# jltsiren/bwt-merge

Measured on AMD Instinct MI355X. Metric: merged Gbases/sec (input1+input2), bit-exact native BWT; value = inputs and result resident in HBM, host_to_host_value = SURVEY 8(d)'s T (page-locked host to page-locked host), higher is better.
Workload: dtype u64

## Files before the change

### bwt-merge_amd/csrc/api/context.hip.h

```cpp
#pragma once


namespace
{

thread_local std::string g_error;

int fail(int code, const char* fmt, ...)
{
  char buf[512];
  va_list ap; va_start(ap, fmt); vsnprintf(buf, sizeof(buf), fmt, ap); va_end(ap);
  g_error = buf;
  return code;
}

inline u64 div_up(u64 a, u64 b) { return (a + b - 1) / b; }

}


struct bwtm_context
{
  int device = -1;
  hipStream_t stream = nullptr;
// ... 3 lines not shown
  std::atomic<long long> live_handles{0};

  bool profiling = false;
  std::string profile_only;
  bool profile_open = false;
  struct Pending { const char* name; hipEvent_t start, stop; };
  std::vector<Pending> pending;
  std::map<std::string, std::pair<double, uint64_t>> totals;
  std::vector<const char*> order;

  std::multimap<u64, void*> free_blocks;
  u64 cached_bytes = 0, held_bytes = 0, peak_bytes = 0;
  struct VBlock { u64 bytes = 0; std::vector<hipMemGenericAllocationHandle_t> chunks; hipEvent_t released = nullptr; };
  bool vmm = false;
  std::vector<hipMemGenericAllocationHandle_t> free_chunks;
  std::map<void*, VBlock> vblocks;
  u64 device_total = 0;
  u64 va_fallbacks = 0;

  void* stream_stage[4] = {nullptr, nullptr, nullptr, nullptr};
  u64 stream_stage_cap[4] = {0, 0, 0, 0};
  u64* host_scratch = nullptr;
  u64 scan1_tiles = 0, pull_scan1_tiles = 0;
  u64 step_forms[3] = {0, 0, 0};
  u64 transcode_forms[16] = {};
};

namespace
{

struct Tuning
{
  long long search_algo = 0;
  long long frontier_unfused = 0;
  long long l1_cap = 0;
  long long emit_path = 0;
  long long round_emits = 1ll << 33;
  long long emit_budget = 0;
  long long frontier_epoch = 512;
  long long eager_cum_budget = 16ll << 30;
  long long upload_chunk = 256ll << 20;
  long long download_chunk = 128ll << 20;
  long long range_ratio = 8;
#ifdef BWTM_EXPERIMENTAL
  long long search_view = 0;
#endif
  long long frontier_stage_out = 1;
  long long frontier_rel = 1;
  long long frontier_parts = 0;
  long long part_capacity = 0;
  long long recs_uniform = 0;
  long long recs_window = 0;
  long long stream_samples_query = 0;
  long long stream_upload = 0;
  long long extract_batch = 1ll << 20;
  long long locate_batch = 1ll << 20;
  long long overlap_batch = 1ll << 20;
  long long approx_batch = 1ll << 16;
  long long correct_batch = 1ll << 20;
  long long ingest_verify = 0;
#ifdef BWTM_DIAGNOSTICS
  long long walk_emit = 0;
  long long walk_blocks = 0;
  long long walk_kernel = 0;
  long long walk_ablate = 0;
  long long walk_variant = 0;
// ... 25 lines not shown
  for(int k = 0; k < 4; k++) { if(c->stream_stage[k]) { (void)hipHostFree(c->stream_stage[k]); } c->stream_stage[k] = nullptr; c->stream_stage_cap[k] = 0; }
}
void apply_env_tuning();

int context_setup(bwtm_context* c, int device)
{
  int count = 0;
  hipError_t e = hipGetDeviceCount(&count);
  if(e != hipSuccess || count <= 0) { return fail(BWTM_ENODEV, "no HIP device available (%s)", hipGetErrorString(e)); }
  if(device < 0 || device >= count) { return fail(BWTM_EINVAL, "device %d out of range (%d devices)", device, count); }
  HIP_TRY(hipSetDevice(device));
  apply_env_tuning();
  c->device = device;
  HIP_TRY(hipStreamCreateWithFlags(&c->stream, hipStreamNonBlocking));
  HIP_TRY(hipStreamCreateWithFlags(&c->copy_stream, hipStreamNonBlocking));
  HIP_TRY(hipHostMalloc((void**)&c->host_scratch, 128 * sizeof(u64), hipHostMallocDefault));
  vmm_setup(c);
  {
    hipDeviceProp_t prop;
    HIP_TRY(hipGetDeviceProperties(&prop, device));
    int per_cu_scan = 0, per_cu_pull = 0;
    HIP_TRY(hipOccupancyMaxActiveBlocksPerMultiprocessor(&per_cu_scan, (const void*)k_frontier_scan1, BLOCK_THREADS, 0));
    HIP_TRY(hipOccupancyMaxActiveBlocksPerMultiprocessor(&per_cu_pull, (const void*)k_pull_scan1, BLOCK_THREADS, 0));
    c->scan1_tiles = std::min<u64>(FRONTIER_SCAN1_TILES, (u64)std::max(per_cu_scan, 0) * (u64)std::max(prop.multiProcessorCount, 0));
    c->pull_scan1_tiles = std::min<u64>(FRONTIER_SCAN1_TILES, (u64)std::max(per_cu_pull, 0) * (u64)std::max(prop.multiProcessorCount, 0));
  }
  HIP_TRY(hipFuncSetAttribute((const void*)k_part_scatter_sorted, hipFuncAttributeMaxDynamicSharedMemorySize, 96 * 1024));
  HIP_TRY(hipFuncSetAttribute((const void*)k_lf_walk_binned<true>, hipFuncAttributeMaxDynamicSharedMemorySize, 40 * 1024));
#ifdef BWTM_DIAGNOSTICS
  HIP_TRY(hipFuncSetAttribute((const void*)k_lf_walk_lds<true>, hipFuncAttributeMaxDynamicSharedMemorySize, 122 * 1024));
  HIP_TRY(hipFuncSetAttribute((const void*)k_lf_walk_lds<false>, hipFuncAttributeMaxDynamicSharedMemorySize, 82 * 1024));
#endif
  return BWTM_OK;
}

void context_teardown(bwtm_context* c)
{
  if(c->device < 0) { return; }
  (void)hipSetDevice(c->device);
  if(c->stream) { (void)hipStreamSynchronize(c->stream); }
  if(c->copy_stream) { (void)hipStreamSynchronize(c->copy_stream); }
  for(auto& p : c->pending) { (void)hipEventDestroy(p.start); (void)hipEventDestroy(p.stop); }
  c->pending.clear();
  pool_trim(c);
  stream_stage_free(c);
  if(c->host_scratch) { (void)hipHostFree(c->host_scratch); }
// ... 40 lines not shown
      ctx->mu.unlock();
    }
  }
  Scope(const Scope&) = delete; Scope& operator=(const Scope&) = delete;
};

#define ENTER(wanted) Scope scope_(wanted); if(scope_.rc != BWTM_OK) { return scope_.rc; }


void profile_begin(const char* name)
{
  CTX.profile_open = (CTX.profiling && (CTX.profile_only.empty() || CTX.profile_only.find(std::string(",") + name + ",") != std::string::npos));
  if(!CTX.profile_open) { return; }
  bwtm_context::Pending p; p.name = name;
  (void)hipEventCreate(&p.start); (void)hipEventCreate(&p.stop);
  (void)hipEventRecord(p.start, CTX.stream);
  CTX.pending.push_back(p);
}

void profile_end()
{
  if(!CTX.profile_open) { return; }
  (void)hipEventRecord(CTX.pending.back().stop, CTX.stream);
}

void profile_collect()
{
  if(CTX.pending.empty()) { return; }
  (void)hipStreamSynchronize(CTX.stream);
  for(auto& p : CTX.pending)
  {
    float ms = 0; (void)hipEventElapsedTime(&ms, p.start, p.stop);
    auto it = CTX.totals.find(p.name);
    if(it == CTX.totals.end()) { CTX.totals[p.name] = std::make_pair((double)ms, (uint64_t)1); CTX.order.push_back(p.name); }
    else { it->second.first += ms; it->second.second += 1; }
    (void)hipEventDestroy(p.start); (void)hipEventDestroy(p.stop);
  }
  CTX.pending.clear();
}

#define LAUNCH_CFG(name, kernel, gridx, gridy, block, lds, ...) do { \
  const unsigned long long gx_ = (unsigned long long)(gridx); \
  if(gx_ * (unsigned long long)(block) >= (1ull << 32)) { return fail(BWTM_EINVAL, "launch of %s: %llu workgroups of %u threads do not fit one grid", name, gx_, (unsigned)(block)); } \
  profile_begin(name); \
  hipLaunchKernelGGL(kernel, dim3((unsigned)gx_, (unsigned)(gridy)), dim3((unsigned)(block)), (unsigned)(lds), CTX.stream, __VA_ARGS__); \
  profile_end(); \
// ... 357 lines not shown
  {
    fail(BWTM_EINVAL, "bwtm_context_destroy: %lld handles of the context are still alive; context not destroyed", context->live_handles.load());
    return;
  }
  context_teardown(context);
  delete context;
}

extern "C" const char* bwtm_last_error(void) { return g_error.c_str(); }

namespace
{
int tune_set(const char* key, long long value)
{
  std::string k(key);
  if(k == "search_algo") { g_tune.search_algo = value; }
  else if(k == "frontier_unfused") { g_tune.frontier_unfused = value; }
  else if(k == "l1_cap") { g_tune.l1_cap = value; }
  else if(k == "emit_path") { g_tune.emit_path = value; }
  else if(k == "round_emits") { g_tune.round_emits = (value > 0 ? value : 1); }
  else if(k == "emit_budget") { g_tune.emit_budget = (value > 0 ? value : 0); }
  else if(k == "frontier_epoch") { g_tune.frontier_epoch = (value > 0 ? value : 512); }
  else if(k == "range_ratio") { g_tune.range_ratio = (value >= 0 ? value : 8); }
#ifdef BWTM_EXPERIMENTAL
  else if(k == "search_view") { g_tune.search_view = (value >= 0 && value <= 2 ? value : 0); }
#endif
  else if(k == "frontier_stage_out") { g_tune.frontier_stage_out = (value != 0); }
  else if(k == "frontier_rel") { g_tune.frontier_rel = (value >= 0 && value <= 2 ? value : 1); }
  else if(k == "frontier_parts") { g_tune.frontier_parts = (value > 0 ? value : 0); }
  else if(k == "stream_samples_query") { g_tune.stream_samples_query = (value != 0); }
  else if(k == "stream_upload") { g_tune.stream_upload = (value != 0); }
  else if(k == "ingest_verify") { g_tune.ingest_verify = (value != 0); }
  else if(k == "extract_batch") { g_tune.extract_batch = (value > 0 ? value : (1ll << 20)); }
  else if(k == "locate_batch") { g_tune.locate_batch = (value > 0 ? std::min<long long>(value, 1ll << 28) : (1ll << 20)); }
  else if(k == "overlap_batch") { g_tune.overlap_batch = (value > 0 ? std::min<long long>(value, 1ll << 28) : (1ll << 20)); }
  else if(k == "approx_batch") { g_tune.approx_batch = (value > 0 ? std::min<long long>(value, 1ll << 28) : (1ll << 16)); }
  else if(k == "correct_batch") { g_tune.correct_batch = (value > 0 ? std::min<long long>(value, 1ll << 28) : (1ll << 20)); }
  else if(k == "part_capacity") { g_tune.part_capacity = value; }
  else if(k == "recs_uniform") { g_tune.recs_uniform = (value > 0 ? 1 : (value < 0 ? -1 : 0)); }
  else if(k == "recs_window") { g_tune.recs_window = (value == 8192 || value == 16384 || value == 32768 ? value : 0); }
  else if(k == "eager_cum_budget") { g_tune.eager_cum_budget = (value > 0 ? value : (16ll << 30)); }
  else if(k == "upload_chunk") { g_tune.upload_chunk = (value > 0 ? value : (256ll << 20)); }
  else if(k == "download_chunk") { g_tune.download_chunk = (value > 0 ? value : (128ll << 20)); }
#ifdef BWTM_DIAGNOSTICS
  else if(k == "walk_emit") { g_tune.walk_emit = value; }
  else if(k == "walk_blocks") { g_tune.walk_blocks = value; }
// ... 165 lines not shown
```

### bwt-merge_amd/csrc/api/search.hip.h

```cpp
#pragma once

struct bwtm_ra
{
  bwtm_context* ctx = nullptr;
  bwtm_ra() : ctx(t_ctx) { if(ctx) { ctx->live_handles++; } }
  ~bwtm_ra() { if(ctx) { ctx->live_handles--; } }
  bwtm_ra(const bwtm_ra&) = delete; bwtm_ra& operator=(const bwtm_ra&) = delete;
  u64 na = 0, nb = 0, n_out = 0;
  u64 nrecs_out = 0, nchunks = 0;
  DevBuf owned_bits;
  void* bits_ptr = nullptr;
  template<class T> T* bits_as() const { return (T*)bits_ptr; }
  DevBuf chunk_base;
  bool finalized = false;
  u64 values = 0;
  bool ranged = false;
  u64 range_first = 0, range_last = 0;
  DevBuf range_rel;
  DevBuf super_boff;
  bool windowed = false;
  u64 win_word_first = 0, win_words = 0;
};

#define WHOLE_RA(ra, who) if((ra)->windowed) { return fail(BWTM_EINVAL, who ": a window of a rank array (bwtm_ra_create_range) only serves the merge over partitioned records and the output-range entry points"); }
// ... 184 lines not shown
  DevBuf segmin; TRY(segmin.alloc(nsteps * nsegs * sizeof(u32)));
  LAUNCH2D("bound_seg_min", k_bound_seg_min, nsegs, nsteps, BLOCK_THREADS, bound.as<const u32>(), ntiles, nsegs, segmin.as<u32>());
  LAUNCH2D("bound_suffix_min", k_bound_suffix_min, nsegs, nsteps, BLOCK_THREADS, bound.as<u32>(), ntiles, nsegs, segmin.as<const u32>(), emit_base.as<const u64>());
  LAUNCH("tile_build", k_tile_build_frontier, ntiles, BLOCK_THREADS, emit16.as<const unsigned short>(), emit_base.as<const u64>(), emit_cap, bound.as<const u32>(),
    ntiles, nsteps, ra->bits_as<u64>() + (tile_first << (TILE_SHIFT - 6)), ra->nchunks * CHUNK_WORDS - (tile_first << (TILE_SHIFT - 6)));
  return BWTM_OK;
}

struct RangeLevels
{
  DevBuf sp[2], r[2], cnt[2], flags, pieces, npieces;
  u64 N = 0, alive = 0, levels = 0;
  u32 piece_cap = 0;
  int cur = 0;
  void release() { for(int k = 0; k < 2; k++) { sp[k].release(); r[k].release(); cnt[k].release(); } flags.release(); pieces.release(); npieces.release(); }
};

int range_phase(const bwtm_index* a, const bwtm_index* b, u64 seq_first, u64 count, bwtm_ra* ra, u64 limit, RangeLevels& L)
{
  const u64 cap = std::min<u64>(5 * limit, count) + 1;
  for(int k = 0; k < 2; k++) { TRY(L.sp[k].alloc(cap * sizeof(u64))); TRY(L.r[k].alloc(cap * sizeof(u64))); TRY(L.cnt[k].alloc(cap * sizeof(u64))); }
  TRY(L.flags.alloc((5 * limit + 1) * sizeof(u64)));
  L.piece_cap = (u32)std::min<u64>(count / 16 + 1024, 1ull << 24);
  TRY(L.pieces.alloc((u64)L.piece_cap * sizeof(RangePiece)));
  TRY(L.npieces.alloc(sizeof(u32), true));
  LAUNCH("range_init", k_range_init, 1, BLOCK_THREADS, L.sp[0].as<u64>(), L.r[0].as<u64>(), L.cnt[0].as<u64>(), seq_first, count, a->m);
  L.N = 1; L.alive = count; L.cur = 0; L.levels = 0;
  while(L.N > 0 && L.N <= limit)
  {
    const int c = L.cur;
    const u64 N = L.N, grid = div_up(N, BLOCK_THREADS);
    LAUNCH("range_step", k_range_step<false>, grid, BLOCK_THREADS, a->view(), b->view(), L.sp[c].as<const u64>(), L.r[c].as<const u64>(), L.cnt[c].as<const u64>(), N,
      L.flags.as<u64>(), (const u64*)nullptr, (u64*)nullptr, (u64*)nullptr, (u64*)nullptr, ra->bits_as<u32>(), L.pieces.as<RangePiece>(), L.npieces.as<u32>(), L.piece_cap);
    LAUNCH("range_emit", k_range_emit, 2048, BLOCK_THREADS, L.pieces.as<const RangePiece>(), L.npieces.as<const u32>(), L.piece_cap, ra->bits_as<u32>());
    HIP_TRY(hipMemsetAsync(L.npieces.p, 0, sizeof(u32), CTX.stream));
    TRY(device_scan<0>(L.flags.as<u64>(), L.flags.as<u64>(), 5 * N + 1));
    LAUNCH("range_children", k_range_step<true>, grid, BLOCK_THREADS, a->view(), b->view(), L.sp[c].as<const u64>(), L.r[c].as<const u64>(), L.cnt[c].as<const u64>(), N,
      (u64*)nullptr, L.flags.as<const u64>(), L.sp[1 - c].as<u64>(), L.r[1 - c].as<u64>(), L.cnt[1 - c].as<u64>(), (u32*)nullptr, (RangePiece*)nullptr, (u32*)nullptr, 0u);
    TRY(fetch_u64(L.flags.as<u64>() + 5 * N, 0));
    HIP_TRY(hipStreamSynchronize(CTX.stream));
    L.N = CTX.host_scratch[0];
    L.cur = 1 - c; L.levels++;
  }
  return BWTM_OK;
}

int range_alive(RangeLevels& L, DevBuf& offsets)
{
  TRY(offsets.alloc((L.N + 1) * sizeof(u64)));
  HIP_TRY(hipMemcpyAsync(offsets.p, L.cnt[L.cur].p, L.N * sizeof(u64), hipMemcpyDeviceToDevice, CTX.stream));
  HIP_TRY(hipMemsetAsync(offsets.as<u64>() + L.N, 0, sizeof(u64), CTX.stream));
  TRY(device_scan<0>(offsets.as<u64>(), offsets.as<u64>(), L.N + 1));
  TRY(fetch_u64(offsets.as<u64>() + L.N, 0));
  HIP_TRY(hipStreamSynchronize(CTX.stream));
  L.alive = CTX.host_scratch[0];
  return BWTM_OK;
}

int range_expand(RangeLevels& L, const DevBuf& offsets, uint2* lo, unsigned short* hi)
{
  const int c = L.cur;
  LAUNCH("range_expand", k_range_expand, div_up(L.N, BLOCK_THREADS), BLOCK_THREADS, L.sp[c].as<const u64>(), L.r[c].as<const u64>(), L.cnt[c].as<const u64>(),
    offsets.as<const u64>(), L.N, lo, hi, L.pieces.as<RangePiece>(), L.npieces.as<u32>(), L.piece_cap);
  LAUNCH("range_expand_pieces", k_range_expand_pieces, 2048, BLOCK_THREADS, L.pieces.as<const RangePiece>(), L.npieces.as<const u32>(), L.piece_cap, lo, hi);
  return BWTM_OK;
}

constexpr u64 FRONTIER_MIN_SEQUENCES = 1ull << 21;

int search_frontier(const bwtm_index* a, const bwtm_index* b, u64 seq_first, u64 count, bwtm_ra* ra)
{
  if(a->n >= (1ull << 40) || b->n >= (1ull << 40) || count >= (1ull << 32)) { return search_partitioned(a, b, seq_first, count, ra); }
  RangeLevels levels;
  DevBuf node_offsets;
  const bool node_phase = (g_tune.range_ratio > 0);
  if(node_phase)
  {
    const u64 limit = std::max<u64>(1, std::min<u64>(count / (u64)g_tune.range_ratio, 1ull << 24));
    TRY(range_phase(a, b, seq_first, count, ra, limit, levels));
    if(levels.N == 0) { return BWTM_OK; }
    TRY(range_alive(levels, node_offsets));
    count = levels.alive;
    if(count == 0) { return BWTM_OK; }
  }
  const u64 ntiles = div_up(ra->n_out + 1, 1ull << TILE_SHIFT);
  const u64 nb_max = div_up(count, FR_BLOCK);
  const u64 nseg = 5 * nb_max;
  const u64 fcap = nb_max * FR_BLOCK;

  const u64 per_seq = b->n / (b->m > 0 ? b->m : 1) + 1;
  u64 emit_budget = (u64)g_tune.emit_budget;
  if(emit_budget == 0)
  {
    emit_budget = 16ull << 30;
    size_t free_b = 0, total_b = 0;
// ... 10 lines not shown
  const u64 bound_budget = 2ull << 30;
  if(EPOCH * (ntiles + 1) * sizeof(u32) > bound_budget) { EPOCH = std::max<u64>(1, bound_budget / ((ntiles + 1) * sizeof(u32))); }

  const bool wide = (a->n >= (1ull << 32) || b->n >= (1ull << 32));
  bool rel = (g_tune.frontier_rel == 2 || (g_tune.frontier_rel == 1 && wide));
  for(int c = 1; c <= 5 && rel; c++) { rel = (a->C[c + 1] - a->C[c] < (1ull << 32) && b->C[c + 1] - b->C[c] < (1ull << 32)); }
#ifdef BWTM_EXPERIMENTAL
  if(g_tune.search_view != 0) { rel = false; }
#endif
  DevBuf lo[2], hi[2], seg_len[2], seg_phys[2], seg_prefix, emit16, emit_base, bound;
  for(int k = 0; k < 2; k++)
  {
    TRY(lo[k].alloc(fcap * 8)); if(wide && (k == 0 || !rel)) { TRY(hi[k].alloc(fcap * 2)); }
    TRY(seg_len[k].alloc((nseg + 1) * sizeof(u64), true)); TRY(seg_phys[k].alloc((nseg + 1) * sizeof(u64), true));
  }
  TRY(seg_prefix.alloc((nseg + 1) * sizeof(u64)));
  DevBuf first_seg; TRY(first_seg.alloc((nb_max + 1) * sizeof(u32)));
  const u32 LOOK = (count >= (1ull << 24) ? 4 : (count >= (1ull << 20) ? 8 : 32));
  struct Events
  {
    hipEvent_t ev[32]; u32 n = 0;
    ~Events() { for(u32 k = 0; k < n; k++) { (void)hipEventDestroy(ev[k]); } }
  } events;
  for(u32 k = 0; k < LOOK; k++) { HIP_TRY(hipEventCreateWithFlags(&events.ev[k], hipEventDisableTiming)); events.n = k + 1; }
  const u64 scan_tiles = div_up(nseg + 1, (u64)SCAN_TILE);
  DevBuf scan_partial; TRY(scan_partial.alloc(scan_tiles * sizeof(u64), true));
  TRY(emit16.alloc((emit_cap + 16) * sizeof(unsigned short)));
  TRY(emit_base.alloc((EPOCH + 1) * sizeof(u64), true));
  TRY(bound.alloc(EPOCH * (ntiles + 1) * sizeof(u32)));
  HIP_TRY(hipMemsetAsync(bound.p, 0xFF, EPOCH * (ntiles + 1) * sizeof(u32), CTX.stream));

  if(node_phase)
  {
    TRY(range_expand(levels, node_offsets, lo[0].as<uint2>(), hi[0].as<unsigned short>()));
    LAUNCH("frontier_init", k_frontier_init_tables, div_up(nseg + 1, BLOCK_THREADS), BLOCK_THREADS, seg_len[0].as<u64>(), seg_phys[0].as<u64>(), nb_max, count);
    levels.release(); node_offsets.release();
  }
  else
  {
    u64 init_items = (fcap > nseg + 1 ? fcap : nseg + 1);
    LAUNCH("frontier_init", k_frontier_init, div_up(init_items, BLOCK_THREADS), BLOCK_THREADS, lo[0].as<uint2>(), hi[0].as<unsigned short>(),
      seg_len[0].as<u64>(), seg_phys[0].as<u64>(), nb_max, seq_first, count, a->m);
  }
  int cur = 0;
  u64 in_epoch = 0;
  u64 alive_bound = count, epoch_used = 0;
#ifdef BWTM_EXPERIMENTAL
  bool use_view = (g_tune.search_view == 1);
  if(g_tune.search_view == 2)
  {
    const u64 steps_left = (b->m > 0 ? b->n / b->m : 0);
    size_t free_b = 0, total_b = 0;
    const u64 need = (num_view_records(a->n) + num_view_records(b->n)) * 64;
    use_view = (count >= (1ull << 22) && steps_left >= 32 && hipMemGetInfo(&free_b, &total_b) == hipSuccess && (u64)free_b + CTX.cached_bytes > need + (8ull << 30));
    (void)hipGetLastError();
  }
  if(use_view)
  {
    int rc_view = ensure_view(a);
    if(rc_view == BWTM_OK) { rc_view = ensure_view(b); }
    if(rc_view != BWTM_OK) { use_view = false; }
  }
#endif
  u64 grid = nb_max;
  u64 written[2] = {nb_max, 0};
  u64* host_ring = nullptr;
  HIP_TRY(hipHostGetDevicePointer((void**)&host_ring, CTX.host_scratch + 64, 0));
  for(u64 t = 0; t <= b->n; t++)
  {
    bool size_in_ring = false;
    if(t >= LOOK)
    {
      HIP_TRY(hipEventSynchronize(events.ev[t % LOOK]));
      alive_bound = CTX.host_scratch[64 + (u32)(t % LOOK)];
      if(alive_bound == 0) { break; }
    }
    if(scan_tiles <= CTX.scan1_tiles && g_tune.frontier_unfused == 0)
    {
      LAUNCH("frontier_scan", k_frontier_scan1, scan_tiles, BLOCK_THREADS, seg_len[cur].as<const u64>(), scan_partial.as<unsigned long long>(), (u32)((t & 0x7FFFFFFFull) + 1), nseg,
        seg_prefix.as<u64>(), first_seg.as<u32>(), emit_base.as<u64>(), in_epoch, host_ring + (t % LOOK));
      size_in_ring = true;
    }
    else if(scan_tiles <= FRONTIER_SCAN_TILES && g_tune.frontier_unfused != 1)
    {
      if(scan_tiles > 1)
      {
        LAUNCH("scan_reduce", k_scan_reduce<0>, scan_tiles, BLOCK_THREADS, seg_len[cur].as<const u64>(), scan_partial.as<u64>(), nseg + 1, (u64)0, scan_tiles);
      }
      LAUNCH("frontier_scan", k_frontier_scan, scan_tiles, BLOCK_THREADS, seg_len[cur].as<const u64>(), scan_partial.as<const u64>(), nseg,
        seg_prefix.as<u64>(), first_seg.as<u32>(), emit_base.as<u64>(), in_epoch, host_ring + (t % LOOK));
      size_in_ring = true;
    }
    else
    {
      TRY(device_scan<0>(seg_len[cur].as<u64>(), seg_prefix.as<u64>(), nseg + 1));
      LAUNCH("frontier_prep", k_frontier_prep, div_up(nseg, BLOCK_THREADS), BLOCK_THREADS, seg_prefix.as<const u64>(), nseg, first_seg.as<u32>(),
        emit_base.as<u64>(), in_epoch);
    }
    if(!size_in_ring) { TRY(fetch_u64(seg_prefix.as<u64>() + nseg, 64 + (u32)(t % LOOK))); HIP_TRY(hipEventRecord(events.ev[t % LOOK], CTX.stream)); }
    {
      const u64 need = std::max<u64>(1, div_up(alive_bound, FR_BLOCK));
      if(g_tune.frontier_parts <= 1 && need * 4 < grid * 3) { grid = need; }
      const int nxt = 1 - cur;
      if(written[nxt] > grid)
      {
        for(u64 c = 0; c < 5; c++) { HIP_TRY(hipMemsetAsync(seg_len[nxt].as<u64>() + c * nb_max + grid, 0, (written[nxt] - grid) * sizeof(u64), CTX.stream)); }
      }
      written[nxt] = grid;
    }
    FrontierView f;
    f.lo = lo[cur].as<const uint2>(); f.hi = hi[cur].as<const unsigned short>();
    f.lo_next = lo[1 - cur].as<uint2>(); f.hi_next = hi[1 - cur].as<unsigned short>();
    f.seg_prefix = seg_prefix.as<const u64>(); f.seg_phys = seg_phys[cur].as<const u64>(); f.first_seg = first_seg.as<const u32>();
// ... 6 lines not shown
    if(g_tune.walk_emit == 1 && wide) { LAUNCH_STEP_REL("frontier_step_noemit", 1, true, rel_form, grid, a->view(), b->view(), f); }
    else if(g_tune.walk_emit == 1) { LAUNCH_STEP_REL("frontier_step_noemit", 1, false, rel_form, grid, a->view(), b->view(), f); }
    else
#endif
    if(g_tune.frontier_parts > 1)
    {
      const u64 parts = (u64)g_tune.frontier_parts, per = div_up(nb_max, parts);
      for(u64 part = 0; part < parts && part * per < nb_max; part++)
      {
        f.block_base = (u32)(part * per);
        const u64 nb_part = std::min<u64>(per, nb_max - part * per);
        const char* label = (part == 0 ? "frontier_step_slice0" : "frontier_step_slices");
        if(wide) { LAUNCH_STEP_REL(label, 0, true, rel_form, nb_part, a->view(), b->view(), f); }
        else { LAUNCH_STEP_REL(label, 0, false, rel_form, nb_part, a->view(), b->view(), f); }
      }
    }
#ifdef BWTM_EXPERIMENTAL
    else if(use_view && wide) { LAUNCH_STEP("frontier_step", 0, true, true, false, grid, a->view(), b->view(), f); }
    else if(use_view) { LAUNCH_STEP("frontier_step", 0, false, true, false, grid, a->view(), b->view(), f); }
#endif
    else if(wide) { LAUNCH_STEP_REL("frontier_step", 0, true, rel_form, grid, a->view(), b->view(), f); }
    else { LAUNCH_STEP_REL("frontier_step", 0, false, rel_form, grid, a->view(), b->view(), f); }
    if(rel && t == 0) { hi[0].release(); }
    if(size_in_ring) { HIP_TRY(hipEventRecord(events.ev[t % LOOK], CTX.stream)); }
    cur = 1 - cur;
    in_epoch++; epoch_used += alive_bound;
    if(in_epoch == EPOCH || (g_tune.l1_cap == 0 && epoch_used + alive_bound > emit_cap))
    {
      TRY(frontier_flush(ra, emit16, emit_cap, emit_base, bound, ntiles, in_epoch));
      HIP_TRY(hipMemsetAsync(bound.p, 0xFF, EPOCH * (ntiles + 1) * sizeof(u32), CTX.stream));
      HIP_TRY(hipMemsetAsync(emit_base.p, 0, (EPOCH + 1) * sizeof(u64), CTX.stream));
      in_epoch = 0; epoch_used = 0;
    }
  }
  TRY(frontier_flush(ra, emit16, emit_cap, emit_base, bound, ntiles, in_epoch));
  return BWTM_OK;
}

}


extern "C" uint64_t bwtm_ra_buffer_bytes(const bwtm_index* a, const bwtm_index* b)
{
  if(!a || !b) { return 0; }
  return div_up(num_records(a->n + b->n), 64) * CHUNK_WORDS * sizeof(u64);
}

// ... 177 lines not shown
```

### bwt-merge_amd/csrc/kernels/search_frontier.hip.h

```cpp
#pragma once


constexpr int FR_BLOCK = 256;
constexpr u32 PULL_SRC_SHIFT_ = 56;
constexpr u64 PULL_PHYS_MASK_ = (1ull << PULL_SRC_SHIFT_) - 1;
constexpr int FR_SEGS = 31;

struct FrontierView
{
  const uint2* lo; const unsigned short* hi;
  uint2* lo_next; unsigned short* hi_next;
  const u64* seg_prefix;
  const u64* seg_phys;
  const u32* first_seg;
  u64* seg_len_next; u64* seg_phys_next;
  u64 nb_max;
  unsigned short* emit16;
  const u64* emit_base;
  u64 emit_cap;
  u32* bits32;
  u32* bound_row;
  u64 step;
  u32 block_base;
  const uint2* const* src_lo; const unsigned short* const* src_hi;
// ... 332 lines not shown
  frontier_step_body<EMIT, HI, VIEW, PULL, STAGE, 0>(A, B, f);
}

template<int REL> struct Rel { static constexpr int value = REL; };
template<class FORM, int EMIT, bool HI, bool STAGE>
__global__ void __launch_bounds__(FR_BLOCK, 8) k_frontier_step(IndexView A, IndexView B, FrontierView f)
{
  frontier_step_body<EMIT, HI, false, false, STAGE, FORM::value>(A, B, f);
}

__global__ void __launch_bounds__(BLOCK_THREADS) k_frontier_prep(const u64* seg_prefix, u64 nseg, u32* first_seg, u64* emit_base, u64 step)
{
  u64 sgm = (u64)blockIdx.x * BLOCK_THREADS + threadIdx.x;
  if(sgm == 0) { emit_base[step + 1] = emit_base[step] + seg_prefix[nseg]; }
  if(sgm >= nseg) { return; }
  u64 begin = seg_prefix[sgm], end = seg_prefix[sgm + 1];
  u64 b = (begin + FR_BLOCK - 1) / FR_BLOCK;
  if(b * FR_BLOCK < end) { first_seg[b] = (u32)sgm; }
}

constexpr u64 FRONTIER_SCAN_TILES = 8192;
constexpr u64 FRONTIER_SCAN1_TILES = 1024;

__global__ void __launch_bounds__(BLOCK_THREADS) k_frontier_scan(const u64* seg_len, const u64* partial, u64 nseg, u64* seg_prefix, u32* first_seg,
  u64* emit_base, u64 step, u64* host_n)
{
  __shared__ u64 lds[BLOCK_THREADS / WAVE];
  const u64 n = nseg + 1;
  u64 c = 0;
  for(u64 k = threadIdx.x; k < blockIdx.x; k += BLOCK_THREADS) { c += partial[k]; }
  const u64 carry = block_reduce<0>(c, lds);
  const u64 base = (u64)blockIdx.x * SCAN_TILE + (u64)threadIdx.x * SCAN_ITEMS;
  u64 item[SCAN_ITEMS];
  u64 acc = 0;
#pragma unroll
  for(int k = 0; k < SCAN_ITEMS; k++) { item[k] = seg_len[base + k < n ? base + k : n - 1]; }
#pragma unroll
  for(int k = 0; k < SCAN_ITEMS; k++) { if(base + k >= n) { item[k] = 0; } acc += item[k]; }
  const u64 incl = wave_incl_sum(acc);
  const u64 wave_total = shfl_u64(incl, WAVE - 1);
  u64 excl = shfl_up_u64(incl, 1);
  if(lane_id() == 0) { excl = 0; }
  if(lane_id() == 0) { lds[threadIdx.x >> 6] = wave_total; }
  __syncthreads();
  u64 run = carry + excl;
  for(int k = 0; k < (int)(threadIdx.x >> 6); k++) { run += lds[k]; }
  for(int k = 0; k < SCAN_ITEMS; k++)
  {
    const u64 idx = base + k;
    if(idx < n)
    {
      seg_prefix[idx] = run;
      if(idx < nseg)
      {
        const u64 b = (run + FR_BLOCK - 1) / FR_BLOCK;
        if(b * FR_BLOCK < run + item[k]) { first_seg[b] = (u32)idx; }
      }
      else { emit_base[step + 1] = emit_base[step] + run; if(host_n) { *host_n = run; } }
    }
    run += item[k];
  }
}

__global__ void __launch_bounds__(BLOCK_THREADS) k_frontier_scan1(const u64* seg_len, unsigned long long* tile_total, u32 tag, u64 nseg, u64* seg_prefix, u32* first_seg,
  u64* emit_base, u64 step, u64* host_n)
{
  __shared__ u64 lds[BLOCK_THREADS / WAVE];
  const u64 n = nseg + 1;
  const u64 base = (u64)blockIdx.x * SCAN_TILE + (u64)threadIdx.x * SCAN_ITEMS;
  u64 item[SCAN_ITEMS];
  u64 acc = 0;
#pragma unroll
  for(int k = 0; k < SCAN_ITEMS; k++) { item[k] = seg_len[base + k < n ? base + k : n - 1]; }
#pragma unroll
  for(int k = 0; k < SCAN_ITEMS; k++) { if(base + k >= n) { item[k] = 0; } acc += item[k]; }
  const u64 incl = wave_incl_sum(acc);
  const u64 wave_total = shfl_u64(incl, WAVE - 1);
  u64 excl = shfl_up_u64(incl, 1);
  if(lane_id() == 0) { excl = 0; }
  if(lane_id() == 0) { lds[threadIdx.x >> 6] = wave_total; }
  __syncthreads();
  u64 before_waves = 0, tile_sum = 0;
  for(int k = 0; k < BLOCK_THREADS / WAVE; k++) { if(k < (int)(threadIdx.x >> 6)) { before_waves += lds[k]; } tile_sum += lds[k]; }
  if(threadIdx.x == 0) { __hip_atomic_store(&tile_total[blockIdx.x], ((unsigned long long)tag << 32) | (unsigned long long)tile_sum, __ATOMIC_RELAXED, __HIP_MEMORY_SCOPE_AGENT); }
  __syncthreads();
  u64 c = 0;
  for(u64 k = threadIdx.x; k < blockIdx.x; k += BLOCK_THREADS)
  {
    unsigned long long w;
    do { w = __hip_atomic_load(&tile_total[k], __ATOMIC_RELAXED, __HIP_MEMORY_SCOPE_AGENT); } while((u32)(w >> 32) != tag);
    c += (u32)w;
  }
  const u64 carry = block_reduce<0>(c, lds);
  u64 run = carry + before_waves + excl;
  for(int k = 0; k < SCAN_ITEMS; k++)
  {
    const u64 idx = base + k;
    if(idx < n)
    {
      seg_prefix[idx] = run;
      if(idx < nseg)
      {
        const u64 b = (run + FR_BLOCK - 1) / FR_BLOCK;
        if(b * FR_BLOCK < run + item[k]) { first_seg[b] = (u32)idx; }
      }
      else { emit_base[step + 1] = emit_base[step] + run; if(host_n) { *host_n = run; } }
    }
    run += item[k];
  }
}

constexpr u32 BOUND_SEG = 2048;

__global__ void __launch_bounds__(BLOCK_THREADS) k_bound_seg_min(const u32* bound, u64 ntiles, u64 nsegs, u32* segmin)
{
  __shared__ u32 lds[BLOCK_THREADS / WAVE];
  const u64 t = blockIdx.y, sg = blockIdx.x;
  const u32* row = bound + t * (ntiles + 1);
  u32 m = 0xFFFFFFFFu;
  for(u64 idx = sg * BOUND_SEG + threadIdx.x; idx < ntiles && idx < (sg + 1) * BOUND_SEG; idx += BLOCK_THREADS) { const u32 v = row[idx]; m = (v < m ? v : m); }
  m = 0xFFFFFFFFu - (u32)wave_max((u64)(0xFFFFFFFFu - m));
  if(lane_id() == 0) { lds[threadIdx.x >> 6] = m; }
  __syncthreads();
  if(threadIdx.x == 0)
  {
    for(int k = 1; k < BLOCK_THREADS / WAVE; k++) { m = (lds[k] < m ? lds[k] : m); }
    segmin[t * nsegs + sg] = m;
  }
}

__global__ void __launch_bounds__(BLOCK_THREADS) k_bound_suffix_min(u32* bound, u64 ntiles, u64 nsegs, const u32* segmin, const u64* emit_base)
{
// ... 173 lines not shown
```

### bwt-merge_amd/csrc/kernels/search_range.hip.h

```cpp
#pragma once

constexpr u32 RANGE_INLINE_WORDS = 4;
constexpr u32 RANGE_PIECE_WORDS = 2048;
constexpr u32 RANGE_EXPAND_INLINE = 48;
constexpr u32 RANGE_EXPAND_PIECE = 1024;

struct RangePiece { u64 first; u64 count; u64 aux; u64 dst; };

__device__ inline void range_set_bits(u32* bits, u64 p0, u64 p1)
{
  for(u64 w = p0 >> 5; w <= ((p1 - 1) >> 5); w++)
  {
    const u64 lo = (w << 5 > p0 ? w << 5 : p0), hi = (((w + 1) << 5) < p1 ? (w + 1) << 5 : p1);
    const u32 n = (u32)(hi - lo), sh = (u32)(lo & 31);
    const u32 mask = (n == 32 ? 0xFFFFFFFFu : ((1u << n) - 1u) << sh);
    atomicOr(bits + w, mask);
  }
}

__global__ void __launch_bounds__(BLOCK_THREADS) k_range_init(u64* sp, u64* r, u64* cnt, u64 seq_first, u64 count, u64 m_a)
{
  if(blockIdx.x == 0 && threadIdx.x == 0) { sp[0] = seq_first; r[0] = m_a; cnt[0] = count; }
}

template<bool WRITE>
__global__ void __launch_bounds__(BLOCK_THREADS) k_range_step(IndexView A, IndexView B, const u64* sp, const u64* r, const u64* cnt, u64 N,
  u64* flags, const u64* prefix, u64* sp_next, u64* r_next, u64* cnt_next, u32* bits, RangePiece* pieces, u32* npieces, u32 piece_cap)
{
  const u64 u = (u64)blockIdx.x * BLOCK_THREADS + threadIdx.x;
  if(u >= N) { return; }
  const u64 s = sp[u], k = cnt[u], rr = r[u];
  u64 rs[6], re[6];
  index_ranks(B, s, rs);
  index_ranks(B, s + k, re);
  if(!WRITE)
  {
#pragma unroll
    for(u32 c = 1; c < 6; c++) { flags[(u64)(c - 1) * N + u] = (re[c] > rs[c] ? 1 : 0); }
    if(u == 0) { flags[5 * N] = 0; }
    const u64 p0 = s + rr, p1 = p0 + k;
    if(((p1 - 1) >> 5) - (p0 >> 5) < RANGE_INLINE_WORDS) { range_set_bits(bits, p0, p1); }
    else
    {
      const u64 per = (u64)RANGE_PIECE_WORDS * 32;
      const u64 first_cut = ((p0 / per) + 1) * per;
      const u32 n = (u32)(p1 <= first_cut ? 1 : 1 + (p1 - first_cut + per - 1) / per);
      const u32 at = atomicAdd(npieces, n);
      u64 b = p0;
      for(u32 q = 0; q < n; q++)
      {
        u64 e = (b / per + 1) * per; if(e > p1) { e = p1; }
        if(at + q < piece_cap) { RangePiece pc; pc.first = b; pc.count = e - b; pc.aux = 0; pc.dst = 0; pieces[at + q] = pc; }
        else { range_set_bits(bits, b, e); }
        b = e;
      }
    }
  }
  else
  {
    u64 ra[6];
    index_ranks(A, rr, ra);
#pragma unroll
    for(u32 c = 1; c < 6; c++)
    {
      if(re[c] > rs[c])
      {
        const u64 d = prefix[(u64)(c - 1) * N + u];
        sp_next[d] = B.C[c] + rs[c];
        cnt_next[d] = re[c] - rs[c];
        r_next[d] = A.C[c] + ra[c];
      }
    }
  }
}

__global__ void __launch_bounds__(BLOCK_THREADS) k_range_emit(const RangePiece* pieces, const u32* npieces, u32 piece_cap, u32* bits)
{
  u32 n = *npieces; if(n > piece_cap) { n = piece_cap; }
  for(u32 q = blockIdx.x; q < n; q += gridDim.x)
  {
    const u64 p0 = pieces[q].first, p1 = p0 + pieces[q].count;
    const u64 w0 = p0 >> 5, w1 = (p1 - 1) >> 5;
    for(u64 w = w0 + threadIdx.x; w <= w1; w += BLOCK_THREADS)
    {
      const u64 lo = (w << 5 > p0 ? w << 5 : p0), hi = (((w + 1) << 5) < p1 ? (w + 1) << 5 : p1);
      const u32 nb = (u32)(hi - lo), sh = (u32)(lo & 31);
      atomicOr(bits + w, (nb == 32 ? 0xFFFFFFFFu : ((1u << nb) - 1u) << sh));
    }
  }
}

__device__ inline void range_store_element(uint2* lo, unsigned short* hi, u64 g, u64 i, u64 r)
{
  lo[g] = make_uint2((u32)i, (u32)r);
  if(hi) { hi[g] = (unsigned short)(((i >> 32) & 0xFF) | (((r >> 32) & 0xFF) << 8)); }
}
// ... 42 lines not shown
```

Before: 93.50.

## Run small range levels in one persistent block and poll tagged frontier sizes

Adds a single-block kernel that advances many small range-search levels in one launch, doing the per-level compaction with in-block scans instead of one launch sequence and host sync per level. Separately, the frontier loop now has the scan kernels publish a tagged size word to pinned host memory with a system-scope store, and the host spin-polls that word instead of recording and synchronizing on events. Both target per-level launch and synchronization latency. The cost is a serial single-workgroup kernel for levels up to the small threshold, host CPU busy-waiting, and extra state to drain the stream before the next search.

```diff
diff --git a/bwt-merge_amd/csrc/api/context.hip.h b/bwt-merge_amd/csrc/api/context.hip.h
--- a/bwt-merge_amd/csrc/api/context.hip.h
+++ b/bwt-merge_amd/csrc/api/context.hip.h
@@ -49,6 +49,7 @@
   u64 stream_stage_cap[4] = {0, 0, 0, 0};
   u64* host_scratch = nullptr;
   u64 scan1_tiles = 0, pull_scan1_tiles = 0;
+  bool ring_in_flight = false;
   u64 step_forms[3] = {0, 0, 0};
   u64 transcode_forms[16] = {};
 };
@@ -56,6 +57,7 @@
 namespace
 {
 
+constexpr long long RANGE_SMALL_DEFAULT = 1024, RANGE_SMALL_MAX = 1ll << 20;
 struct Tuning
 {
   long long search_algo = 0;
@@ -69,6 +71,9 @@
   long long upload_chunk = 256ll << 20;
   long long download_chunk = 128ll << 20;
   long long range_ratio = 8;
+  long long range_small = RANGE_SMALL_DEFAULT;
+  long long range_piece_cap = 0;
+  long long frontier_poll = 1;
 #ifdef BWTM_EXPERIMENTAL
   long long search_view = 0;
 #endif
@@ -140,6 +145,9 @@
     int per_cu_scan = 0, per_cu_pull = 0;
     HIP_TRY(hipOccupancyMaxActiveBlocksPerMultiprocessor(&per_cu_scan, (const void*)k_frontier_scan1, BLOCK_THREADS, 0));
     HIP_TRY(hipOccupancyMaxActiveBlocksPerMultiprocessor(&per_cu_pull, (const void*)k_pull_scan1, BLOCK_THREADS, 0));
+    int per_cu_tagged = 0;
+    HIP_TRY(hipOccupancyMaxActiveBlocksPerMultiprocessor(&per_cu_tagged, (const void*)k_frontier_scan1_tagged, BLOCK_THREADS, 0));
+    per_cu_scan = std::min(per_cu_scan, per_cu_tagged);
     c->scan1_tiles = std::min<u64>(FRONTIER_SCAN1_TILES, (u64)std::max(per_cu_scan, 0) * (u64)std::max(prop.multiProcessorCount, 0));
     c->pull_scan1_tiles = std::min<u64>(FRONTIER_SCAN1_TILES, (u64)std::max(per_cu_pull, 0) * (u64)std::max(prop.multiProcessorCount, 0));
   }
@@ -226,6 +234,15 @@
 {
   if(!CTX.profile_open) { return; }
   (void)hipEventRecord(CTX.pending.back().stop, CTX.stream);
+}
+
+void profile_add_count(const char* name, uint64_t n)
+{
+  if(n == 0 || !CTX.profiling) { return; }
+  if(!CTX.profile_only.empty() && CTX.profile_only.find(std::string(",") + name + ",") == std::string::npos) { return; }
+  auto it = CTX.totals.find(name);
+  if(it == CTX.totals.end()) { CTX.totals[name] = std::make_pair(0.0, n); CTX.order.push_back(name); }
+  else { it->second.second += n; }
 }
 
 void profile_collect()
@@ -629,6 +646,9 @@
   else if(k == "emit_budget") { g_tune.emit_budget = (value > 0 ? value : 0); }
   else if(k == "frontier_epoch") { g_tune.frontier_epoch = (value > 0 ? value : 512); }
   else if(k == "range_ratio") { g_tune.range_ratio = (value >= 0 ? value : 8); }
+  else if(k == "range_small") { g_tune.range_small = (value >= 0 ? std::min<long long>(value, RANGE_SMALL_MAX) : RANGE_SMALL_DEFAULT); }
+  else if(k == "range_piece_cap") { g_tune.range_piece_cap = (value > 0 ? std::min<long long>(value, 1ll << 24) : 0); }
+  else if(k == "frontier_poll") { g_tune.frontier_poll = (value == 0 ? 0 : 1); }
 #ifdef BWTM_EXPERIMENTAL
   else if(k == "search_view") { g_tune.search_view = (value >= 0 && value <= 2 ? value : 0); }
 #endif
diff --git a/bwt-merge_amd/csrc/api/search.hip.h b/bwt-merge_amd/csrc/api/search.hip.h
--- a/bwt-merge_amd/csrc/api/search.hip.h
+++ b/bwt-merge_amd/csrc/api/search.hip.h
@@ -230,10 +230,31 @@
   for(int k = 0; k < 2; k++) { TRY(L.sp[k].alloc(cap * sizeof(u64))); TRY(L.r[k].alloc(cap * sizeof(u64))); TRY(L.cnt[k].alloc(cap * sizeof(u64))); }
   TRY(L.flags.alloc((5 * limit + 1) * sizeof(u64)));
   L.piece_cap = (u32)std::min<u64>(count / 16 + 1024, 1ull << 24);
+  if(g_tune.range_piece_cap > 0) { L.piece_cap = (u32)g_tune.range_piece_cap; }
   TRY(L.pieces.alloc((u64)L.piece_cap * sizeof(RangePiece)));
   TRY(L.npieces.alloc(sizeof(u32), true));
   LAUNCH("range_init", k_range_init, 1, BLOCK_THREADS, L.sp[0].as<u64>(), L.r[0].as<u64>(), L.cnt[0].as<u64>(), seq_first, count, a->m);
   L.N = 1; L.alive = count; L.cur = 0; L.levels = 0;
+  const u64 small = std::min<u64>(limit, (u64)g_tune.range_small);
+  if(small > 0)
+  {
+    DevBuf state; TRY(state.alloc(3 * sizeof(u64)));
+    const u32 max_levels = (u32)std::min<u64>(b->n - b->m + 2, 1u << 16);
+    while(L.N > 0 && L.N <= small)
+    {
+      LAUNCH("range_small", k_range_small, 1, RANGE_SMALL_THREADS, a->view(), b->view(), L.sp[0].as<u64>(), L.r[0].as<u64>(), L.cnt[0].as<u64>(),
+        L.sp[1].as<u64>(), L.r[1].as<u64>(), L.cnt[1].as<u64>(), L.N, (u32)L.cur, count, small, max_levels, ra->bits_as<u32>(),
+        L.pieces.as<RangePiece>(), L.npieces.as<u32>(), L.piece_cap, state.as<u64>());
+      LAUNCH("range_emit", k_range_emit, 2048, BLOCK_THREADS, L.pieces.as<const RangePiece>(), L.npieces.as<const u32>(), L.piece_cap, ra->bits_as<u32>());
+      HIP_TRY(hipMemsetAsync(L.npieces.p, 0, sizeof(u32), CTX.stream));
+      TRY(fetch_u64(state.as<u64>(), 0, 3));
+      HIP_TRY(hipStreamSynchronize(CTX.stream));
+      const u64 done = CTX.host_scratch[1];
+      if(done == 0) { return fail(BWTM_ENODEV, "bwtm_search: the node kernel processed no level (%llu nodes)", (unsigned long long)L.N); }
+      L.N = CTX.host_scratch[0]; L.cur = (int)CTX.host_scratch[2]; L.levels += done;
+      profile_add_count("range_step", done); profile_add_count("range_children", done);
+    }
+  }
   while(L.N > 0 && L.N <= limit)
   {
     const int c = L.cur;
@@ -276,9 +297,31 @@
 
 constexpr u64 FRONTIER_MIN_SEQUENCES = 1ull << 21;
 
+inline u32 ring_tag(u64 t) { return (u32)((t + 1) & 0xFFFFFFFFull); }
+
+inline int ring_verdict(u64 word, u32 tag, hipError_t stream_state, u64* n)
+{
+  if((u32)(word >> 32) == tag) { *n = word & 0xFFFFFFFFull; return 1; }
+  return (stream_state == hipErrorNotReady ? 0 : -1);
+}
+
+int ring_wait(const u64* slot, u32 tag, hipStream_t stream, u64* n)
+{
+  for(u64 looks = 1; ; looks++)
+  {
+    hipError_t state = hipErrorNotReady;
+    if((looks & 4095) == 0) { state = hipStreamQuery(stream); if(state != hipSuccess) { (void)hipGetLastError(); } }
+    const u64 word = __atomic_load_n(slot, __ATOMIC_ACQUIRE);
+    const int v = ring_verdict(word, tag, state, n);
+    if(v > 0) { return BWTM_OK; }
+    if(v < 0) { return fail(BWTM_ENODEV, "bwtm_search: the frontier's size never arrived (stream: %s)", state == hipSuccess ? "idle" : hipGetErrorString(state)); }
+  }
+}
+
 int search_frontier(const bwtm_index* a, const bwtm_index* b, u64 seq_first, u64 count, bwtm_ra* ra)
 {
   if(a->n >= (1ull << 40) || b->n >= (1ull << 40) || count >= (1ull << 32)) { return search_partitioned(a, b, seq_first, count, ra); }
+  if(CTX.ring_in_flight) { HIP_TRY(hipStreamSynchronize(CTX.stream)); CTX.ring_in_flight = false; }
   RangeLevels levels;
   DevBuf node_offsets;
   const bool node_phase = (g_tune.range_ratio > 0);
@@ -335,8 +378,10 @@
     hipEvent_t ev[32]; u32 n = 0;
     ~Events() { for(u32 k = 0; k < n; k++) { (void)hipEventDestroy(ev[k]); } }
   } events;
-  for(u32 k = 0; k < LOOK; k++) { HIP_TRY(hipEventCreateWithFlags(&events.ev[k], hipEventDisableTiming)); events.n = k + 1; }
   const u64 scan_tiles = div_up(nseg + 1, (u64)SCAN_TILE);
+  const bool scan_writes_ring = ((scan_tiles <= CTX.scan1_tiles && g_tune.frontier_unfused == 0) || (scan_tiles <= FRONTIER_SCAN_TILES && g_tune.frontier_unfused != 1));
+  const bool poll = (g_tune.frontier_poll != 0 && scan_writes_ring);
+  if(!poll) { for(u32 k = 0; k < LOOK; k++) { HIP_TRY(hipEventCreateWithFlags(&events.ev[k], hipEventDisableTiming)); events.n = k + 1; } }
   DevBuf scan_partial; TRY(scan_partial.alloc(scan_tiles * sizeof(u64), true));
   TRY(emit16.alloc((emit_cap + 16) * sizeof(unsigned short)));
   TRY(emit_base.alloc((EPOCH + 1) * sizeof(u64), true));
@@ -379,19 +424,32 @@
   u64 written[2] = {nb_max, 0};
   u64* host_ring = nullptr;
   HIP_TRY(hipHostGetDevicePointer((void**)&host_ring, CTX.host_scratch + 64, 0));
+  if(poll)
+  {
+    for(u32 k = 0; k < LOOK; k++) { __atomic_store_n(CTX.host_scratch + 64 + k, (u64)0, __ATOMIC_RELAXED); }
+    CTX.ring_in_flight = true;
+  }
   for(u64 t = 0; t <= b->n; t++)
   {
     bool size_in_ring = false;
     if(t >= LOOK)
     {
-      HIP_TRY(hipEventSynchronize(events.ev[t % LOOK]));
-      alive_bound = CTX.host_scratch[64 + (u32)(t % LOOK)];
+      if(poll) { TRY(ring_wait(CTX.host_scratch + 64 + (u32)(t % LOOK), ring_tag(t - LOOK), CTX.stream, &alive_bound)); }
+      else { HIP_TRY(hipEventSynchronize(events.ev[t % LOOK])); alive_bound = CTX.host_scratch[64 + (u32)(t % LOOK)]; }
       if(alive_bound == 0) { break; }
     }
     if(scan_tiles <= CTX.scan1_tiles && g_tune.frontier_unfused == 0)
     {
-      LAUNCH("frontier_scan", k_frontier_scan1, scan_tiles, BLOCK_THREADS, seg_len[cur].as<const u64>(), scan_partial.as<unsigned long long>(), (u32)((t & 0x7FFFFFFFull) + 1), nseg,
-        seg_prefix.as<u64>(), first_seg.as<u32>(), emit_base.as<u64>(), in_epoch, host_ring + (t % LOOK));
+      if(poll)
+      {
+        LAUNCH("frontier_scan", k_frontier_scan1_tagged, scan_tiles, BLOCK_THREADS, seg_len[cur].as<const u64>(), scan_partial.as<unsigned long long>(), (u32)((t & 0x7FFFFFFFull) + 1), nseg,
+          seg_prefix.as<u64>(), first_seg.as<u32>(), emit_base.as<u64>(), in_epoch, host_ring + (t % LOOK), (u64)ring_tag(t));
+      }
+      else
+      {
+        LAUNCH("frontier_scan", k_frontier_scan1, scan_tiles, BLOCK_THREADS, seg_len[cur].as<const u64>(), scan_partial.as<unsigned long long>(), (u32)((t & 0x7FFFFFFFull) + 1), nseg,
+          seg_prefix.as<u64>(), first_seg.as<u32>(), emit_base.as<u64>(), in_epoch, host_ring + (t % LOOK));
+      }
       size_in_ring = true;
     }
     else if(scan_tiles <= FRONTIER_SCAN_TILES && g_tune.frontier_unfused != 1)
@@ -400,8 +458,16 @@
       {
         LAUNCH("scan_reduce", k_scan_reduce<0>, scan_tiles, BLOCK_THREADS, seg_len[cur].as<const u64>(), scan_partial.as<u64>(), nseg + 1, (u64)0, scan_tiles);
       }
-      LAUNCH("frontier_scan", k_frontier_scan, scan_tiles, BLOCK_THREADS, seg_len[cur].as<const u64>(), scan_partial.as<const u64>(), nseg,
-        seg_prefix.as<u64>(), first_seg.as<u32>(), emit_base.as<u64>(), in_epoch, host_ring + (t % LOOK));
+      if(poll)
+      {
+        LAUNCH("frontier_scan", k_frontier_scan_tagged, scan_tiles, BLOCK_THREADS, seg_len[cur].as<const u64>(), scan_partial.as<const u64>(), nseg,
+          seg_prefix.as<u64>(), first_seg.as<u32>(), emit_base.as<u64>(), in_epoch, host_ring + (t % LOOK), (u64)ring_tag(t));
+      }
+      else
+      {
+        LAUNCH("frontier_scan", k_frontier_scan, scan_tiles, BLOCK_THREADS, seg_len[cur].as<const u64>(), scan_partial.as<const u64>(), nseg,
+          seg_prefix.as<u64>(), first_seg.as<u32>(), emit_base.as<u64>(), in_epoch, host_ring + (t % LOOK));
+      }
       size_in_ring = true;
     }
     else
@@ -454,7 +520,7 @@
     else if(wide) { LAUNCH_STEP_REL("frontier_step", 0, true, rel_form, grid, a->view(), b->view(), f); }
     else { LAUNCH_STEP_REL("frontier_step", 0, false, rel_form, grid, a->view(), b->view(), f); }
     if(rel && t == 0) { hi[0].release(); }
-    if(size_in_ring) { HIP_TRY(hipEventRecord(events.ev[t % LOOK], CTX.stream)); }
+    if(size_in_ring && !poll) { HIP_TRY(hipEventRecord(events.ev[t % LOOK], CTX.stream)); }
     cur = 1 - cur;
     in_epoch++; epoch_used += alive_bound;
     if(in_epoch == EPOCH || (g_tune.l1_cap == 0 && epoch_used + alive_bound > emit_cap))
diff --git a/bwt-merge_amd/csrc/kernels/search_frontier.hip.h b/bwt-merge_amd/csrc/kernels/search_frontier.hip.h
--- a/bwt-merge_amd/csrc/kernels/search_frontier.hip.h
+++ b/bwt-merge_amd/csrc/kernels/search_frontier.hip.h
@@ -378,8 +378,15 @@
 constexpr u64 FRONTIER_SCAN_TILES = 8192;
 constexpr u64 FRONTIER_SCAN1_TILES = 1024;
 
-__global__ void __launch_bounds__(BLOCK_THREADS) k_frontier_scan(const u64* seg_len, const u64* partial, u64 nseg, u64* seg_prefix, u32* first_seg,
-  u64* emit_base, u64 step, u64* host_n)
+__device__ inline void frontier_publish_size(u64* host_n, u64 host_tag, u64 n_t)
+{
+  if(!host_n) { return; }
+  if(host_tag == 0) { *host_n = n_t; return; }
+  __hip_atomic_store((unsigned long long*)host_n, (unsigned long long)((host_tag << 32) | n_t), __ATOMIC_RELAXED, __HIP_MEMORY_SCOPE_SYSTEM);
+}
+
+__device__ inline void frontier_scan_body(const u64* seg_len, const u64* partial, u64 nseg, u64* seg_prefix, u32* first_seg,
+  u64* emit_base, u64 step, u64* host_n, u64 host_tag)
 {
   __shared__ u64 lds[BLOCK_THREADS / WAVE];
   const u64 n = nseg + 1;
@@ -412,14 +419,26 @@
         const u64 b = (run + FR_BLOCK - 1) / FR_BLOCK;
         if(b * FR_BLOCK < run + item[k]) { first_seg[b] = (u32)idx; }
       }
-      else { emit_base[step + 1] = emit_base[step] + run; if(host_n) { *host_n = run; } }
+      else { emit_base[step + 1] = emit_base[step] + run; frontier_publish_size(host_n, host_tag, run); }
     }
     run += item[k];
   }
 }
 
-__global__ void __launch_bounds__(BLOCK_THREADS) k_frontier_scan1(const u64* seg_len, unsigned long long* tile_total, u32 tag, u64 nseg, u64* seg_prefix, u32* first_seg,
+__global__ void __launch_bounds__(BLOCK_THREADS) k_frontier_scan(const u64* seg_len, const u64* partial, u64 nseg, u64* seg_prefix, u32* first_seg,
   u64* emit_base, u64 step, u64* host_n)
+{
+  frontier_scan_body(seg_len, partial, nseg, seg_prefix, first_seg, emit_base, step, host_n, 0);
+}
+
+__global__ void __launch_bounds__(BLOCK_THREADS) k_frontier_scan_tagged(const u64* seg_len, const u64* partial, u64 nseg, u64* seg_prefix, u32* first_seg,
+  u64* emit_base, u64 step, u64* host_n, u64 host_tag)
+{
+  frontier_scan_body(seg_len, partial, nseg, seg_prefix, first_seg, emit_base, step, host_n, host_tag);
+}
+
+__device__ inline void frontier_scan1_body(const u64* seg_len, unsigned long long* tile_total, u32 tag, u64 nseg, u64* seg_prefix, u32* first_seg,
+  u64* emit_base, u64 step, u64* host_n, u64 host_tag)
 {
   __shared__ u64 lds[BLOCK_THREADS / WAVE];
   const u64 n = nseg + 1;
@@ -460,10 +479,22 @@
         const u64 b = (run + FR_BLOCK - 1) / FR_BLOCK;
         if(b * FR_BLOCK < run + item[k]) { first_seg[b] = (u32)idx; }
       }
-      else { emit_base[step + 1] = emit_base[step] + run; if(host_n) { *host_n = run; } }
+      else { emit_base[step + 1] = emit_base[step] + run; frontier_publish_size(host_n, host_tag, run); }
     }
     run += item[k];
   }
+}
+
+__global__ void __launch_bounds__(BLOCK_THREADS) k_frontier_scan1(const u64* seg_len, unsigned long long* tile_total, u32 tag, u64 nseg, u64* seg_prefix, u32* first_seg,
+  u64* emit_base, u64 step, u64* host_n)
+{
+  frontier_scan1_body(seg_len, tile_total, tag, nseg, seg_prefix, first_seg, emit_base, step, host_n, 0);
+}
+
+__global__ void __launch_bounds__(BLOCK_THREADS) k_frontier_scan1_tagged(const u64* seg_len, unsigned long long* tile_total, u32 tag, u64 nseg, u64* seg_prefix, u32* first_seg,
+  u64* emit_base, u64 step, u64* host_n, u64 host_tag)
+{
+  frontier_scan1_body(seg_len, tile_total, tag, nseg, seg_prefix, first_seg, emit_base, step, host_n, host_tag);
 }
 
 constexpr u32 BOUND_SEG = 2048;
diff --git a/bwt-merge_amd/csrc/kernels/search_range.hip.h b/bwt-merge_amd/csrc/kernels/search_range.hip.h
--- a/bwt-merge_amd/csrc/kernels/search_range.hip.h
+++ b/bwt-merge_amd/csrc/kernels/search_range.hip.h
@@ -15,6 +15,24 @@
     const u32 n = (u32)(hi - lo), sh = (u32)(lo & 31);
     const u32 mask = (n == 32 ? 0xFFFFFFFFu : ((1u << n) - 1u) << sh);
     atomicOr(bits + w, mask);
+  }
+}
+
+__device__ inline void range_run_bits(u32* bits, u64 p0, u64 k, RangePiece* pieces, u32* npieces, u32 piece_cap)
+{
+  const u64 p1 = p0 + k;
+  if(((p1 - 1) >> 5) - (p0 >> 5) < RANGE_INLINE_WORDS) { range_set_bits(bits, p0, p1); return; }
+  const u64 per = (u64)RANGE_PIECE_WORDS * 32;
+  const u64 first_cut = ((p0 / per) + 1) * per;
+  const u32 n = (u32)(p1 <= first_cut ? 1 : 1 + (p1 - first_cut + per - 1) / per);
+  const u32 at = atomicAdd(npieces, n);
+  u64 b = p0;
+  for(u32 q = 0; q < n; q++)
+  {
+    u64 e = (b / per + 1) * per; if(e > p1) { e = p1; }
+    if(at + q < piece_cap) { RangePiece pc; pc.first = b; pc.count = e - b; pc.aux = 0; pc.dst = 0; pieces[at + q] = pc; }
+    else { range_set_bits(bits, b, e); }
+    b = e;
   }
 }
 
@@ -38,23 +56,7 @@
 #pragma unroll
     for(u32 c = 1; c < 6; c++) { flags[(u64)(c - 1) * N + u] = (re[c] > rs[c] ? 1 : 0); }
     if(u == 0) { flags[5 * N] = 0; }
-    const u64 p0 = s + rr, p1 = p0 + k;
-    if(((p1 - 1) >> 5) - (p0 >> 5) < RANGE_INLINE_WORDS) { range_set_bits(bits, p0, p1); }
-    else
-    {
-      const u64 per = (u64)RANGE_PIECE_WORDS * 32;
-      const u64 first_cut = ((p0 / per) + 1) * per;
-      const u32 n = (u32)(p1 <= first_cut ? 1 : 1 + (p1 - first_cut + per - 1) / per);
-      const u32 at = atomicAdd(npieces, n);
-      u64 b = p0;
-      for(u32 q = 0; q < n; q++)
-      {
-        u64 e = (b / per + 1) * per; if(e > p1) { e = p1; }
-        if(at + q < piece_cap) { RangePiece pc; pc.first = b; pc.count = e - b; pc.aux = 0; pc.dst = 0; pieces[at + q] = pc; }
-        else { range_set_bits(bits, b, e); }
-        b = e;
-      }
-    }
+    range_run_bits(bits, s + rr, k, pieces, npieces, piece_cap);
   }
   else
   {
@@ -72,6 +74,108 @@
       }
     }
   }
+}
+
+constexpr u32 RANGE_SMALL_THREADS = 1024;
+constexpr u32 RANGE_SMALL_FIELD = 12;
+
+__device__ inline u64 range_small_uniform(u64 v)
+{
+  return ((u64)(u32)__builtin_amdgcn_readfirstlane((int)(u32)(v >> 32)) << 32) | (u64)(u32)__builtin_amdgcn_readfirstlane((int)(u32)v);
+}
+
+__device__ inline u64 range_small_load(const u64* p) { return __hip_atomic_load(p, __ATOMIC_RELAXED, __HIP_MEMORY_SCOPE_AGENT); }
+
+__device__ inline u64 range_small_field(u64 packed, u32 c) { return (packed >> (RANGE_SMALL_FIELD * (c - 1))) & ((1ull << RANGE_SMALL_FIELD) - 1); }
+
+__global__ void __launch_bounds__(RANGE_SMALL_THREADS) k_range_small(IndexView A, IndexView B, u64* sp0, u64* r0, u64* cnt0, u64* sp1, u64* r1, u64* cnt1,
+  u64 N, u32 cur, u64 alive, u64 small, u32 max_levels, u32* bits, RangePiece* pieces, u32* npieces, u32 piece_cap, u64* state)
+{
+  __shared__ u64 wave_total[RANGE_SMALL_THREADS / WAVE];
+  __shared__ u32 sym_total[6];
+  const u32 tid = threadIdx.x, wave = tid >> 6;
+  u32 levels = 0;
+  while(N > 0 && N <= small && levels < max_levels)
+  {
+    const u32 have = __hip_atomic_load(npieces, __ATOMIC_RELAXED, __HIP_MEMORY_SCOPE_AGENT);
+    if(have > 0 && (u64)have + 2 * N + alive / ((u64)RANGE_PIECE_WORDS * 32) + 1 > (u64)piece_cap) { break; }
+    const u64* sp = (cur ? sp1 : sp0); const u64* r = (cur ? r1 : r0); const u64* cnt = (cur ? cnt1 : cnt0);
+    u64* sp_next = (cur ? sp0 : sp1); u64* r_next = (cur ? r0 : r1); u64* cnt_next = (cur ? cnt0 : cnt1);
+    const u64 nchunks = (N + RANGE_SMALL_THREADS - 1) / RANGE_SMALL_THREADS;
+    u64 tot[6] = {0, 0, 0, 0, 0, 0};
+    if(nchunks > 1)
+    {
+      if(tid < 6) { sym_total[tid] = 0; }
+      __syncthreads();
+      u32 mine[6] = {0, 0, 0, 0, 0, 0};
+      for(u64 chunk = 0; chunk < nchunks; chunk++)
+      {
+        const u64 u = chunk * RANGE_SMALL_THREADS + tid;
+        const bool valid = (u < N);
+        u64 rs[6] = {0, 0, 0, 0, 0, 0}, re[6] = {0, 0, 0, 0, 0, 0};
+        if(valid) { const u64 s = range_small_load(sp + u); index_ranks(B, s, rs); index_ranks(B, s + range_small_load(cnt + u), re); }
+#pragma unroll
+        for(u32 c = 1; c < 6; c++) { mine[c] += (u32)__popcll(__ballot(re[c] > rs[c])); }
+      }
+      if(lane_id() == 0)
+      {
+#pragma unroll
+        for(u32 c = 1; c < 6; c++) { atomicAdd(&sym_total[c], mine[c]); }
+      }
+      __syncthreads();
+#pragma unroll
+      for(u32 c = 1; c < 6; c++) { tot[c] = range_small_uniform(sym_total[c]); }
+    }
+    u64 carry[6] = {0, 0, 0, 0, 0, 0};
+    for(u64 chunk = 0; chunk < nchunks; chunk++)
+    {
+      const u64 u = chunk * RANGE_SMALL_THREADS + tid;
+      const bool valid = (u < N);
+      u64 rs[6] = {0, 0, 0, 0, 0, 0}, re[6] = {0, 0, 0, 0, 0, 0}, ra[6] = {0, 0, 0, 0, 0, 0};
+      if(valid)
+      {
+        const u64 s = range_small_load(sp + u), k = range_small_load(cnt + u), rr = range_small_load(r + u);
+        range_run_bits(bits, s + rr, k, pieces, npieces, piece_cap);
+        index_ranks(B, s, rs);
+        index_ranks(B, s + k, re);
+        index_ranks(A, rr, ra);
+      }
+      u64 packed = 0;
+#pragma unroll
+      for(u32 c = 1; c < 6; c++) { packed |= (u64)(re[c] > rs[c] ? 1 : 0) << (RANGE_SMALL_FIELD * (c - 1)); }
+      const u64 incl = wave_incl_sum(packed);
+      if(lane_id() == WAVE - 1) { wave_total[wave] = incl; }
+      __syncthreads();
+      u64 before = incl - packed, chunk_total = 0;
+      for(u32 k = 0; k < RANGE_SMALL_THREADS / WAVE; k++) { const u64 w = wave_total[k]; if(k < wave) { before += w; } chunk_total += w; }
+      chunk_total = range_small_uniform(chunk_total);
+      __syncthreads();
+      if(nchunks == 1)
+      {
+#pragma unroll
+        for(u32 c = 1; c < 6; c++) { tot[c] = range_small_field(chunk_total, c); }
+      }
+      u64 base = 0;
+#pragma unroll
+      for(u32 c = 1; c < 6; c++)
+      {
+        if(re[c] > rs[c])
+        {
+          const u64 d = base + carry[c] + range_small_field(before, c);
+          sp_next[d] = B.C[c] + rs[c];
+          cnt_next[d] = re[c] - rs[c];
+          r_next[d] = A.C[c] + ra[c];
+        }
+        base += tot[c];
+        carry[c] += range_small_field(chunk_total, c);
+      }
+    }
+    N = tot[1] + tot[2] + tot[3] + tot[4] + tot[5];
+    cur ^= 1u; levels++;
+    __builtin_amdgcn_fence(__ATOMIC_RELEASE, "workgroup");
+    __syncthreads();
+  }
+  if(tid == 0) { state[0] = N; state[1] = levels; state[2] = cur; }
 }
 
 __global__ void __launch_bounds__(BLOCK_THREADS) k_range_emit(const RangePiece* pieces, const u32* npieces, u32 piece_cap, u32* bits)
```

Result: no change. 93.68 (median of 5 runs) (+0.2%).
